# jakovdev/SequenceAligner

Hardware: AMD Instinct MI355X
Metric: pair-alignments/sec (higher is better)
Workload: dtype u16x2; 1 GPU; cfg2: 10000 protein seqs x U[80,120], nw blosum62 {'gap_pen': 4}, all-vs-all packed triangular; pairs=49995000, cells=501594494441, parallelism=pair-range x1

## Files before the change

sequencealigner_amd/csrc/sa_context.hip:

```cpp
#include <algorithm>
#include <cmath>
#include <cstdio>
#include <cstdlib>
#include <cstring>

#include "sa_ctx.h"

bool sa_device_ready(int device)
{
	int count = 0;
	hipError_t err = hipGetDeviceCount(&count);
	if (err != hipSuccess || count <= 0) {
		sa_set_error("No HIP devices available (%s); libseqalign_hip has no CPU fallback",
			     err == hipSuccess ? "device count is 0" : hipGetErrorString(err));
		return false;
	}
	if (device < 0 || device >= count) {
		sa_set_error("HIP device %d out of range (%d visible)", device, count);
		return false;
	}
	SA_HIP_CHECK(hipSetDevice(device), return false);
	return true;
}

// ... 237 lines not shown
	return sa_guard("sa_ctx_create", (sa_ctx *)nullptr, [&] { return ctx_create_impl(device, in, sc); });
}

extern "C" void sa_ctx_destroy(sa_ctx *ctx)
{
	if (!ctx)
		return;
	(void)hipSetDevice(ctx->device);
	for (auto &ev : ctx->events) {
		(void)hipEventDestroy(ev.e0);
		(void)hipEventDestroy(ev.e1);
	}
	sa_plan_release(ctx);
	sa_deliver_release(ctx);
	for (auto &ar : ctx->arranged) {
		(void)hipFree(ar.d_codes);
		(void)hipFree(ar.d_off);
		(void)hipFree(ar.d_rowmap);
		(void)hipFree(ar.d_posmap);
		(void)hipFree(ar.d_tok);
		(void)hipFree(ar.d_tok_off);
		(void)hipFree(ar.d_mine);
		(void)hipFree(ar.d_any);
	}
	(void)hipFree(ctx->d_codes);
	(void)hipFree(ctx->d_meta);
	(void)hipFree(ctx->d_off);
	(void)hipFree(ctx->d_sub);
	(void)hipFree(ctx->d_sub8);
	(void)hipFree(ctx->d_scratch);
	(void)hipFree(ctx->d_id_scratch);
	(void)hipFree(ctx->d_counters);
	for (hipEvent_t ev : ctx->slot_done)
		if (ev)
			(void)hipEventDestroy(ev);
	(void)hipFree(ctx->d_long_scratch);
	delete ctx;
}

extern "C" int64_t sa_ctx_pairs(const sa_ctx *ctx) { return ctx ? ctx->pairs : -1; }
bool sa_arranged_store(sa_ctx *ctx, const SaArrKey &key, const sa_ctx::Arranged **out)
{
	*out = nullptr;
	for (const auto &ar : ctx->arranged)
		if (ar.key == key) {
			*out = &ar;
// ... 24 lines not shown
		return false;
	sa_ctx::Arranged ar;
	ar.key = key;
	bool ok = false;
	do {
		if (!ts.tok.empty()) {
			SA_HIP_CHECK(hipMalloc(&ar.d_tok, sizeof(uint16_t) * ts.tok.size()), break);
			SA_HIP_CHECK(hipMalloc(&ar.d_tok_off, sizeof(int32_t) * ts.tok_off.size()), break);
			SA_HIP_CHECK(hipMalloc(&ar.d_mine, sizeof(uint16_t) * ts.mine.size()), break);
			SA_HIP_CHECK(hipMalloc(&ar.d_any, sizeof(uint16_t) * ts.any.size()), break);
			SA_HIP_CHECK(hipMemcpy(ar.d_tok, ts.tok.data(), sizeof(uint16_t) * ts.tok.size(), hipMemcpyHostToDevice), break);
			SA_HIP_CHECK(hipMemcpy(ar.d_tok_off, ts.tok_off.data(), sizeof(int32_t) * ts.tok_off.size(), hipMemcpyHostToDevice), break);
			SA_HIP_CHECK(hipMemcpy(ar.d_mine, ts.mine.data(), sizeof(uint16_t) * ts.mine.size(), hipMemcpyHostToDevice), break);
			SA_HIP_CHECK(hipMemcpy(ar.d_any, ts.any.data(), sizeof(uint16_t) * ts.any.size(), hipMemcpyHostToDevice), break);
		}
		SA_HIP_CHECK(hipMalloc(&ar.d_codes, codes_s.size()), break);
		SA_HIP_CHECK(hipMalloc(&ar.d_off, sizeof(int32_t) * off_s.size()), break);
		SA_HIP_CHECK(hipMalloc(&ar.d_rowmap, sizeof(int32_t) * rowmap.size()), break);
		SA_HIP_CHECK(hipMalloc(&ar.d_posmap, sizeof(int32_t) * posmap.size()), break);
		SA_HIP_CHECK(hipMemcpy(ar.d_codes, codes_s.data(), codes_s.size(), hipMemcpyHostToDevice), break);
		SA_HIP_CHECK(hipMemcpy(ar.d_off, off_s.data(), sizeof(int32_t) * off_s.size(), hipMemcpyHostToDevice), break);
		SA_HIP_CHECK(hipMemcpy(ar.d_rowmap, rowmap.data(), sizeof(int32_t) * rowmap.size(), hipMemcpyHostToDevice), break);
		SA_HIP_CHECK(hipMemcpy(ar.d_posmap, posmap.data(), sizeof(int32_t) * posmap.size(), hipMemcpyHostToDevice), break);
		ctx->arranged.push_back(ar);
		ok = true;
	} while (0);
	if (!ok) {
		(void)hipFree(ar.d_codes);
		(void)hipFree(ar.d_off);
		(void)hipFree(ar.d_rowmap);
		(void)hipFree(ar.d_posmap);
		(void)hipFree(ar.d_tok);
		(void)hipFree(ar.d_tok_off);
		(void)hipFree(ar.d_mine);
		(void)hipFree(ar.d_any);
		return false;
	}
	*out = &ctx->arranged.back();
	return true;
}

extern "C" void sa_ctx_timing(sa_ctx *ctx, int enable)
{
	if (!ctx)
		return;
	(void)hipSetDevice(ctx->device);
	for (auto &ev : ctx->events) {
		(void)hipEventDestroy(ev.e0);
		(void)hipEventDestroy(ev.e1);
	}
	ctx->events.clear();
	ctx->timing = enable != 0;
}

static int timing_read_impl(sa_ctx *ctx, char *kernel_name, int cap, int64_t *launches, double *total_ms,
			    int64_t *pairs, int64_t *cells, double *all_kernels_ms)
{
	if (!ctx)
		return 1;
	(void)hipSetDevice(ctx->device);
	struct Acc {
// ... 48 lines not shown
```

sequencealigner_amd/csrc/sa_ctx.h:

```cpp
#ifndef SA_CTX_H
#define SA_CTX_H

#include <atomic>
#include <chrono>
#include <deque>
#include <exception>
#include <memory>
#include <new>
#include <string>
#include <vector>

#include "sa_env.h"
#include "sa_guard.h"
#include "sa_internal.h"
#include "sa_plan.h"

struct sa_ctx {
	int device = 0;
	int32_t num = 0, max_len = 0, min_len = 0;
	int64_t pairs = 0;
	sa_scoring sc{};
	SaEnv env;
	std::vector<sa_meta> meta;
	std::vector<int32_t> off;
// ... 10 lines not shown
	enum { COUNTER_SLOTS = 256, COUNTERS_PER_SLOT = 2 * SA_PLAN_NCLASSES };
	unsigned *d_counters = nullptr;
	uint64_t call_no = 0;
	hipEvent_t slot_done[COUNTER_SLOTS] = {};
	bool slot_dirty[COUNTER_SLOTS] = {};
	int32_t *d_long_scratch = nullptr;
	int64_t long_stride = 0;
	int long_wgs = 0;
	int persistent_wgs = 0;
	bool sys_ok = false;
	int32_t sys_pconst = 0, sys_q = 0;
	int64_t sys_gain = 0, sys_slack = 0;
	int pk_kmax = 0, pk16_kmax = 0;
	int pk16_f16_kmax = 0;
	int pk_chunk_cap = SA_SYS_CHUNK;
	int32_t pk_pconst = 0, pk_q = 0, pk_floor = 0;
	int64_t pk_gain = 0, pk_slack = 0, pk_extra = 0;
	struct Arranged {
		SaArrKey key;
		uint8_t *d_codes = nullptr;
		int32_t *d_off = nullptr, *d_rowmap = nullptr, *d_posmap = nullptr;
		uint16_t *d_tok = nullptr, *d_mine = nullptr, *d_any = nullptr;
		int32_t *d_tok_off = nullptr;
	};
	std::deque<Arranged> arranged;
	int64_t tok_lean = 0, tok_legacy = 0;
	bool out_is_host = false;
	struct Plan {
		SaHostPlan h;
		struct DevClass {
			int32_t *d_jlist = nullptr, *d_tprefix = nullptr, *d_tlist = nullptr;
			int64_t *d_doff = nullptr;
		};
		struct DevBundle {
			SaPkClassArgs *d_args = nullptr;
			uint32_t *d_ulist = nullptr;
		};
		std::vector<DevClass> dc;
		std::vector<DevBundle> db;
		SaPlaceSeg *d_segs = nullptr;
		int32_t nsegs = 0;
		uint64_t stamp = 0;
	};
	std::vector<std::unique_ptr<Plan>> plans;
	Plan *plan = nullptr;
	uint64_t plan_clock = 0;
// ... 14 lines not shown
		double encode = 0, device = 0, upload = 0, code_objects = 0, pin = 0, plan = 0, arrange = 0;
	} setup;
	struct Deliver {
		hipStream_t compute = nullptr, copy = nullptr;
		hipEvent_t done[2] = {}, copied[2] = {};
		int32_t *d_buf[2] = {};
		int64_t buf_elems[2] = {};
		int32_t *h_stage[2] = {};
		int64_t stage_elems[2] = {};
		int32_t *d_packed = nullptr, *d_full = nullptr;
		int64_t packed_elems = 0, full_elems = 0;
		unsigned *h_counters = nullptr;
		int64_t h_counters_n = 0;
	} dl;
};

static inline double sa_ms_since(std::chrono::steady_clock::time_point t0)
{
	return std::chrono::duration<double, std::milli>(std::chrono::steady_clock::now() - t0).count();
}

bool sa_device_ready(int device);
bool sa_arranged_store(sa_ctx *ctx, const SaArrKey &key, const sa_ctx::Arranged **out);
SaPlanInputs sa_plan_inputs(const sa_ctx *ctx);

void sa_plan_release(sa_ctx *ctx);
bool sa_plan_get(sa_ctx *ctx, int64_t start, int64_t count, int world, bool share_host);
bool sa_prepare_range(sa_ctx *ctx, int64_t start, int64_t count, bool host_out);
int sa_align_range_impl(sa_ctx *ctx, int64_t start, int64_t count, int32_t *d_scores, void *stream, bool out16,
			int world = 0, int rank = 0, int32_t *host_out = nullptr);

void sa_deliver_release(sa_ctx *ctx);
bool sa_host_range_is_pinned(const void *p, size_t bytes);
size_t sa_host_available_bytes();
bool sa_host_range_in_malloc_heap(const void *p, size_t bytes);

bool sa_progress_wanted();
void sa_report_progress(double fraction);
void sa_progress_speaker(bool here);
int sa_devices_in_use(const SaEnv &env);

bool sa_align_gathered(struct sa_input in, struct sa_output out, const struct sa_scoring *sc, const int *devices, int ndev,
		       double *phase_seconds, double *breakdown_ms);
bool sa_rccl_available(std::string *why);

bool sa_norm_check(const char *who, const struct sa_norm *norm);
// ... 7 lines not shown
```

sequencealigner_amd/csrc/sa_launch.hip:

```cpp
#include <algorithm>
#include <cstdio>
#include <cstring>

#include "sa_ctx.h"


static void plan_free_device(sa_ctx::Plan &pl)
{
	for (auto &c : pl.dc) {
		(void)hipFree(c.d_jlist);
		(void)hipFree(c.d_tprefix);
		(void)hipFree(c.d_tlist);
		(void)hipFree(c.d_doff);
	}
	(void)hipFree(pl.d_segs);
	for (auto &b : pl.db) {
		(void)hipFree(b.d_args);
		(void)hipFree(b.d_ulist);
	}
	pl.dc.clear();
	pl.db.clear();
	pl.d_segs = nullptr;
}

void sa_plan_release(sa_ctx *ctx)
{
	for (auto &pl : ctx->plans)
		plan_free_device(*pl);
	ctx->plans.clear();
	ctx->plan = nullptr;
}

template <typename T> static bool upload(T *&dst, const std::vector<T> &v)
{
	SA_HIP_CHECK(hipMalloc(reinterpret_cast<void **>(&dst), sizeof(T) * std::max<size_t>(v.size(), 1)), return false);
	if (!v.empty()) {
		SA_HIP_CHECK(hipMemcpy(dst, v.data(), sizeof(T) * v.size(), hipMemcpyHostToDevice), return false);
	}
	return true;
}

static bool resolve_levels(sa_ctx *ctx, const SaArrKey (&keys)[SA_PK_SORT_LEVELS], SaArranged (&lv)[SA_PK_SORT_LEVELS])
{
	for (int l = 0; l < SA_PK_SORT_LEVELS; l++) {
		lv[l] = SaArranged{};
		if (!keys[l].block)
			continue;
		const sa_ctx::Arranged *ar = nullptr;
		if (!sa_arranged_store(ctx, keys[l], &ar))
			return false;
		if (ar)
			lv[l] = { ar->d_codes, ar->d_off, ar->d_rowmap, ar->d_posmap, ar->key.block, ar->d_tok, ar->d_tok_off, ar->d_mine, ar->d_any };
	}
	return true;
}

static bool plan_upload(sa_ctx *ctx, sa_ctx::Plan &pl)
{
	const SaHostPlan &h = pl.h;
	pl.dc.resize(h.classes.size());
	for (size_t ci = 0; ci < h.classes.size(); ci++) {
		const auto &cl = h.classes[ci];
		auto &d = pl.dc[ci];
		if (!upload(d.d_jlist, cl.jlist) || !upload(d.d_tprefix, cl.tprefix))
			return false;
		if (h.world >= 1 && (!upload(d.d_tlist, cl.tlist) || !upload(d.d_doff, cl.doff)))
			return false;
	}
	if (h.world >= 1 && !h.segs.empty()) {
		std::vector<SaPlaceSeg> segs(h.segs.size());
		for (size_t k = 0; k < h.segs.size(); k++) {
			const SaHostSeg &hs = h.segs[k];
			SaPlaceSeg &sg = segs[k];
			sg = SaPlaceSeg{};
			sg.src = hs.src;
// ... 7 lines not shown
			if (hs.map_kind) {
				const sa_ctx::Arranged *ar = nullptr;
				if (!sa_arranged_store(ctx, hs.key, &ar))
					return false;
				if (!ar) {
					sa_set_error("plan: placement names an arranged copy the store does not have");
					return false;
				}
				sg.map = hs.map_kind == 2 ? ar->d_posmap : ar->d_rowmap;
			}
		}
		if (!upload(pl.d_segs, segs))
			return false;
		pl.nsegs = (int32_t)segs.size();
	}
	pl.db.resize(h.bundles.size());
	for (size_t bi = 0; bi < h.bundles.size(); bi++) {
		const auto &b = h.bundles[bi];
		std::vector<SaPkClassArgs> args(b.args.size());
		for (size_t x = 0; x < b.args.size(); x++) {
			const SaHostPkArgs &ha = b.args[x];
			SaPkClassArgs &a = args[x];
			a = SaPkClassArgs{};
			if (!resolve_levels(ctx, ha.lv, a.lv))
				return false;
			const auto &d = pl.dc[(size_t)ha.cls_index];
			a.jlist = d.d_jlist;
			a.tprefix = d.d_tprefix;
			a.dense_off = h.world >= 1 ? d.d_doff : nullptr;
			a.ncols = ha.ncols;
			a.npart = ha.npart;
			a.k = ha.k;
			a.delta = ha.delta;
			a.pk_base = ha.pk_base;
			a.chunk = ha.chunk;
		}
		if (!upload(pl.db[bi].d_args, args) || !upload(pl.db[bi].d_ulist, b.ulist))
			return false;
	}
	return true;
}

bool sa_plan_get(sa_ctx *ctx, int64_t start, int64_t count, int world, bool share_host)
{
	for (auto &pl : ctx->plans)
		if (pl->h.start == start && pl->h.count == count && pl->h.world == world && pl->h.share_host == share_host) {
			pl->stamp = ++ctx->plan_clock;
// ... 544 lines not shown
```

sequencealigner_amd/csrc/sa_plan.cpp:

```cpp
#include "sa_plan.h"
#include "sa_guard.h"

#include <algorithm>
#include <cmath>
#include <cstdlib>

int32_t sa_column_of(int64_t p)
{
	int64_t j = (int64_t)((1.0 + std::sqrt(1.0 + 8.0 * (double)p)) * 0.5);
	while (j * (j - 1) / 2 > p)
		--j;
	while ((j + 1) * j / 2 <= p)
		++j;
	return (int32_t)j;
}

SaPairPlan::SaPairPlan(const sa_meta *m, int32_t n) : num(n), pairs((int64_t)n * (n - 1) / 2), meta(m)
{
	len_prefix.assign((size_t)n + 1, 0);
	cell_prefix.assign((size_t)n + 1, 0);
	for (int32_t k = 0; k < n; k++) {
		len_prefix[(size_t)k + 1] = len_prefix[(size_t)k] + m[k].len;
		cell_prefix[(size_t)k + 1] = cell_prefix[(size_t)k] + (int64_t)m[k].len * len_prefix[(size_t)k];
	}
// ... 133 lines not shown
			sa_set_error("token streams: store too large for 32-bit stream offsets");
			return false;
		}
	}
	ts.tok_off[(size_t)streams] = (int32_t)total;
	ts.tok.assign((size_t)total, (uint16_t)SA_CODE_NOP);
	ts.mine.assign((size_t)(total / 16), 0);
	ts.any.assign((size_t)(total / 16 / ng), 0);
	for (int32_t s = 0; s < streams; s++) {
		const int32_t b = off[(size_t)s * ch], n = off[(size_t)(s + 1) * ch] - b, at = ts.tok_off[(size_t)s];
		const int32_t any_at = ts.tok_off[(size_t)(s / ng * ng)] / 16 / ng;
		for (int32_t p = 0; p < n; p++) {
			const uint8_t c = codes[(size_t)b + (size_t)p];
			ts.tok[(size_t)at + (size_t)p] = c;
			if (c == SA_CODE_SEP) {
				ts.mine[(size_t)(at / 16 + p / 16)] |= (uint16_t)(1u << (p & 15));
				ts.any[(size_t)(any_at + p / 16)] |= (uint16_t)(1u << (p & 15));
			}
		}
	}
	return true;
}

static const char *const TOO_LARGE = "packed range too large for one launch; split it into smaller ranges";

bool sa_plan_host(const SaPlanInputs &in, int64_t start, int64_t count, int world, bool share_host, SaHostPlan &plan)
{
	plan = SaHostPlan();
	const int32_t num = in.num;
	const int64_t all_pairs = (int64_t)num * (num - 1) / 2;
	if (num < 2 || !in.meta || start < 0 || count <= 0 || start > all_pairs - count || world < 0 || world > 1024) {
		sa_set_error("plan: bad range [%lld,+%lld) of %lld pairs or world %d", (long long)start, (long long)count,
			     (long long)all_pairs, world);
		return false;
	}
	const int64_t end = start + count;
	std::vector<std::vector<int32_t>> jl((size_t)SA_PLAN_NCLASSES), tp((size_t)SA_PLAN_NCLASSES);
	std::vector<int64_t> cpairs((size_t)SA_PLAN_NCLASSES, 0), ccells((size_t)SA_PLAN_NCLASSES, 0);
	std::vector<std::vector<std::pair<int32_t, int32_t>>> rows_of((size_t)SA_PLAN_NCLASSES);
	std::vector<int64_t> lenpre((size_t)num + 1, 0);
	for (int32_t k = 0; k < num; k++)
		lenpre[(size_t)k + 1] = lenpre[(size_t)k] + in.meta[k].len;
	{
		const int64_t want_tiles = (int64_t)in.persistent_wgs * 6;
		const int64_t mine = world > 1 ? count / world : count;
		int32_t chunk = SA_SYS_CHUNK;
		while (chunk > 8 && mine / (4 * chunk) < want_tiles)
// ... 423 lines not shown
```

sequencealigner_amd/csrc/sa_plan.h:

```cpp
#ifndef SA_PLAN_H
#define SA_PLAN_H

#include <cstdint>
#include <string>
#include <utility>
#include <vector>

#include "sa_shapes.h"

int32_t sa_column_of(int64_t p);
inline int64_t sa_tri(int64_t j) { return j * (j - 1) / 2; }

struct SaPairPlan {
	int32_t num = 0;
	int64_t pairs = 0;
	const sa_meta *meta = nullptr;
	std::vector<int64_t> len_prefix;
	std::vector<int64_t> cell_prefix;
	SaPairPlan(const sa_meta *m, int32_t n);
	int64_t cells_before(int64_t p) const;
};

struct SaArrKey {
	int ng = 0, ch = 0;
// ... 31 lines not shown

int32_t sa_pk_delta(const SaPlanInputs &in, int g, int k);
int32_t sa_pk_base(const SaPlanInputs &in, int g, int k);

struct SaPkCls {
	bool small;
	int g, k;
};
SaPkCls sa_pk_decode(int cls);
int sa_systolic_class_for(int32_t n);

bool sa_arranged_exists(int32_t num, const SaArrKey &key);
int sa_pk_arranged_keys(const SaPlanInputs &in, int pk_g, int pk_k, int32_t chunk_pk, bool host_out, SaArrKey (&lv)[SA_PK_SORT_LEVELS]);
void sa_arrange_rows(const sa_meta *meta, int32_t num, const SaArrKey &key, std::vector<int32_t> &rowmap);

struct SaTokenStreams {
	int32_t streams = 0;
	std::vector<uint16_t> tok, mine, any;
	std::vector<int32_t> tok_off;
};
inline int32_t sa_token_blocks(int32_t smax, int g) { return ((smax + g - 1 + 15) >> 4) + 2; }
bool sa_build_tokens(const uint8_t *codes, const int32_t *off, int32_t num, const SaArrKey &key, SaTokenStreams &ts);

struct SaHostClass {
	int cls = 0;
	int32_t ncols = 0, ntiles = 0;
	int32_t npart = 0;
	int32_t chunk = 0;
	int64_t pairs = 0, cells = 0;
	std::vector<int32_t> jlist, tprefix;
	std::vector<int32_t> part_rows;
	std::vector<int32_t> tlist;
	std::vector<int64_t> doff;
	std::vector<int16_t> owner;
	std::vector<int32_t> rank_first;
	std::vector<int64_t> rank_pairs, rank_cells;
};

struct SaHostSeg {
	int64_t src, dst;
	int32_t count, pos0, ia, ib, flags;
	int map_kind;
	SaArrKey key;
};

struct SaHostPkArgs {
// ... 40 lines not shown
```

sequencealigner_amd/csrc/sa_shapes.h:

```cpp
#ifndef SA_SHAPES_H
#define SA_SHAPES_H

#include <cstdint>

#include "../../include/seqalign_hip.h"

#if defined(__HIPCC__)
#define SA_HD __host__ __device__
#else
#define SA_HD
#endif

enum : int { SA_CODE_SEP = 24, SA_CODE_NOP = 25, SA_CODE_ROWS = 26 };

void sa_set_error(const char *fmt, ...) __attribute__((format(printf, 1, 2)));


#define SA_SYS_CHUNK 32
#define SA_SYS_WPB(G, LONG) ((G) >= 32 ? 4 : 1)
#define SA_SYS_CLASS_LIST(X) \
	X(0, 8, 1) X(1, 8, 2) X(2, 8, 3) X(3, 8, 4) \
	X(4, 8, 5) X(5, 8, 6) X(6, 8, 7) X(7, 8, 8) \
	X(8, 8, 9) X(9, 8, 10) X(10, 8, 11) X(11, 8, 12) \
	X(12, 8, 13) X(13, 8, 14) X(14, 8, 15) X(15, 8, 16) \
// ... 23 lines not shown
}
#define SA_PK_F16_MAX 0x7bff
#define SA_PK_ROWS_OWN_BLOCK 1024
#define SA_PK_SORT_LEVELS 4
#define SA_PK_SORT_ROWS 2048
#define SA_PK_KMAX 24
#define SA_PK_K_LIST(X) \
	X(1) X(2) X(3) X(4) X(5) X(6) X(7) X(8) X(9) X(10) X(11) X(12) \
	X(13) X(14) X(15) X(16) X(17) X(18) X(19) X(20) X(21) X(22) X(23) X(24)
#define SA_PK_K16_MIN 13
#define SA_PK16_KMAX 64
#define SA_PK16_F16_KMAX 52
#define SA_PK_K16_LIST(X) \
	X(13) X(14) X(15) X(16) X(17) X(18) X(19) X(20) X(21) X(22) X(23) X(24) X(25) X(26) \
	X(27) X(28) X(29) X(30) X(31) X(32) X(33) X(34) X(35) X(36) X(37) X(38) X(39) X(40) \
	X(41) X(42) X(43) X(44) X(45) X(46) X(47) X(48) X(49) X(50) X(51) X(52) X(53) X(54) \
	X(55) X(56) X(57) X(58) X(59) X(60) X(61) X(62) X(63) X(64)
enum : int { SA_PK_CLASS0 = SA_SYS_NCLASSES + 1, SA_PK16_CLASS0 = SA_PK_CLASS0 + SA_PK_KMAX + 1,
	     SA_PK_CLASSES_END = SA_PK16_CLASS0 + SA_PK16_KMAX + 1,
	     SA_PK_SMALL = SA_PK_CLASSES_END - SA_PK_CLASS0,
	     SA_PLAN_NCLASSES = SA_PK_CLASSES_END + SA_PK_SMALL };

#define SA_PK_BUNDLE 8
struct SaArranged {
	const uint8_t *codes;
	const int32_t *off;
	const int32_t *rowmap;
	const int32_t *posmap;
	int32_t rows;
	const uint16_t *tok;
	const int32_t *tok_off;
	const uint16_t *mine;
	const uint16_t *any;
};
struct SaPkClassArgs {
	const int32_t *jlist;
	const int32_t *tprefix;
	const int64_t *dense_off;
	int32_t ncols, npart, k;
	int32_t delta, pk_base;
	int32_t chunk;
	SaArranged lv[SA_PK_SORT_LEVELS];
};
#define SA_PK_UTILE_BITS 28
SA_HD constexpr int sa_pk_lds_fixed(int g, int wpb) { return 416 * wpb * (64 / g); }
SA_HD constexpr int sa_pk_lds_bytes(int method, int g, int k) { return sa_pk_lds_fixed(g, sa_pk_wpb(method, g, k)) + SA_CODE_ROWS * ((k + 3) / 4) * 256; }
inline int sa_pk_bundle_klo(int g, int k) { return g == 8 ? 1 + (k - 1) / SA_PK_BUNDLE * SA_PK_BUNDLE : SA_PK_K16_MIN + (k - SA_PK_K16_MIN) / SA_PK_BUNDLE * SA_PK_BUNDLE; }


#define SA_SHARE_PAD(rows) (((rows) + 7) & ~7)

SA_HD inline int sa_pk_pick_level(const int32_t *lvrows, int32_t ra, int32_t rb, int32_t i_begin, int32_t tile_rows)
{
	int pick = -1;
	if (ra % tile_rows != 0)
		return pick;
// ... 22 lines not shown
```

sequencealigner_amd/csrc/sa_systolic_pk.inc:

```
#include "sa_internal.h"
#include <atomic>
#include <type_traits>
#if !defined(SA_PK_G) || (SA_PK_G != 8 && SA_PK_G != 16)
#error "define SA_PK_G (8 or 16) before including sa_systolic_pk.inc"
#endif
#if SA_PK_G == 16 && !defined(SA_PK16_PART)
#error "define SA_PK16_PART (0: K = 13..44, 1: K = 45..64) before including sa_systolic_pk.inc with SA_PK_G 16"
#endif

#define SA_PK_STORE(nt, v, p)                          \
	do {                                           \
		if (nt) {                              \
			asm volatile("");  \
			__builtin_nontemporal_store((v), (p)); \
		} else                                 \
			*(p) = (v);                    \
	} while (0)

#ifndef SA_PK_OPAQUE_TOKEN
#define SA_PK_OPAQUE_TOKEN 1
#endif
#ifndef SA_PK_PAIRED_ADDS
#define SA_PK_PAIRED_ADDS 1
#endif
// ... 156 lines not shown
	for (int h = 0; h < 2; h++) {
		const int32_t j = jh[h];
		tri[h] = (int64_t)j * (j - 1) / 2;
		const int64_t a = A.start > tri[h] ? A.start - tri[h] : 0;
		const int64_t b = A.end - tri[h] < j ? A.end - tri[h] : j;
		ia[h] = (int32_t)a;
		ib[h] = (int32_t)(b > a ? b : a);
		offj[h] = uload(A.off + j);
		nh[h] = uload(A.off + j + 1) - offj[h] - 1;
		pad[h] = W - nh[h];
	}
	const int32_t ra = ia[0] < ia[1] ? ia[0] : ia[1], rb = ib[0] > ib[1] ? ib[0] : ib[1];
	const int32_t chunk = t < nfull ? t - uload(A.tprefix + lo) : uload(A.tprefix + lo + 1) - uload(A.tprefix + lo);
	const int32_t ch_full = A.chunk;
	const int32_t i_begin = ra + chunk * (NGW * ch_full);
	const int32_t i_count = rb - i_begin < NGW * ch_full ? rb - i_begin : NGW * ch_full;
	const int32_t ch = (i_count + NGW - 1) / NGW;
	const int gw = wv * NG;
	const uint8_t *rcodes = A.codes;
	const int32_t *roff = A.off, *rowmap = nullptr, *posmap = nullptr;
	int32_t sort_rows = 0;
	const uint16_t *tk_tok = nullptr, *tk_mine = nullptr, *tk_any = nullptr;
	const int32_t *tk_off = nullptr;
	{
		const int32_t lvrows[SA_PK_SORT_LEVELS] = { uload(&A.lvp[0].rows), uload(&A.lvp[1].rows), uload(&A.lvp[2].rows),
							    uload(&A.lvp[3].rows) };
		static_assert(SA_PK_SORT_LEVELS == 4, "lvrows lists four levels");
		const int l = sa_pk_pick_level(lvrows, ra, rb, i_begin, NGW * ch_full);
		if (l >= 0) {
			const SaArranged &L = A.lvp[l];
			rcodes = uniform_ptr(L.codes);
			roff = uniform_ptr(L.off);
			rowmap = uniform_ptr(L.rowmap);
			posmap = uniform_ptr(L.posmap);
			tk_tok = uniform_ptr(L.tok);
			tk_off = uniform_ptr(L.tok_off);
			tk_mine = uniform_ptr(L.mine);
			tk_any = uniform_ptr(L.any);
			sort_rows = lvrows[0];
#pragma unroll
			for (int k = 1; k < SA_PK_SORT_LEVELS; k++)
				if (l == k)
					sort_rows = lvrows[k];
		}
	}
	const bool sorted = sort_rows > 0;

	int8_t *const sub = reinterpret_cast<int8_t *>(s_out_all);
	for (int k = lane_id; k < SA_SUB_DIM * SA_SUB_DIM; k += 64 * WPB)
		sub[k] = A.sub8[k];
	uint8_t *const s_cols = reinterpret_cast<uint8_t *>(s_ring_all);
	static_assert(2 * W <= WPB * NG * GSTRIDE * 2, "the staged columns fit the ring storage");
	for (int k = lane_id; k < 2 * W; k += 64 * WPB) {
		const int h = k >= W, c0 = k - h * W - pad[h];
		s_cols[k] = c0 >= 0 ? A.codes[offj[h] + c0] : (uint8_t)0xff;
	}
	__syncthreads();

	{
		constexpr int BUILDERS = NGW / COPIES;
		constexpr int ROWS_EACH = (SA_CODE_ROWS + BUILDERS - 1) / BUILDERS;
// ... 69 lines not shown
	auto fold16 = [&](unsigned long long m) -> uint32_t {
		m |= m >> 32;
		m |= m >> 16;
		return (uint32_t)m & 0xffffu;
	};
	auto block_events = [&](const uint32_t (&w)[TPL], uint32_t &mine) -> uint32_t {
		if (G == 16) {
			const unsigned long long m = __ballot(w[0] == SEPWORD);
			mine = (uint32_t)(m >> (lane & 48)) & 0xffffu;
			return fold16(m);
		}
		uint32_t any = 0;
		mine = 0;
#pragma unroll
		for (int u = 0; u < TPL; u++) {
			const unsigned long long m = __ballot(w[u] == SEPWORD);
			const uint32_t f = fold16(m);
			any |= ((f | (f >> 1)) & 0x5555u) << u;
			mine |= ((uint32_t)(m >> ((lane & 48) + (lane & 1))) & 0x5555u) << u;
		}
		return any;
	};

	const int32_t lean = __builtin_amdgcn_readfirstlane(tk_tok != nullptr ? 1 : 0);
	const uint16_t *tk_any_w = nullptr;
	if (lean) {
		const int32_t s0 = i_begin / ch_full + gw;
		const uint32_t o_w = (uint32_t)uload(tk_off + s0), o_g = (uint32_t)tk_off[s0 + grp];
		bw_a = 2u * o_g + (G == 8 ? 4u * (uint32_t)(r16 >> 1) : 2u * (uint32_t)r16);
		bw_b = o_g >> 3;
		tk_any_w = tk_any + (o_w >> 4) / NG;
		bw_c = (uint32_t)(WPB * OUT_HALFS * 2 + 2 * (wv * (NG * GSTRIDE) + grp * GSTRIDE + fpos(0)));
	}
	auto lean_load = [&](int32_t blk) -> uint32_t {
		const uint8_t *const b = reinterpret_cast<const uint8_t *>(tk_tok) + (size_t)(uint32_t)(blk << 5);
		asm volatile("" : "+v"(bw_a));
		return *reinterpret_cast<const tok_t *>(b + bw_a);
	};
	auto lean_mine = [&](int32_t blk) -> uint32_t {
		const uint8_t *const b = reinterpret_cast<const uint8_t *>(tk_mine) + (size_t)(uint32_t)(blk << 1);
		asm volatile("" : "+v"(bw_b));
		return *reinterpret_cast<const uint16_t *>(b + bw_b);
	};
	auto lean_any = [&](int32_t blk) -> uint32_t { return (uint32_t)tk_any_w[blk]; };
	auto lean_any_s = [&](uint32_t v) -> uint32_t { return (uint32_t)__builtin_amdgcn_readfirstlane((int)v); };
	auto lean_ring = [&](int32_t blk, uint32_t raw) {
		const uint32_t w = __umul24(raw, TUNIT);
		tok_t *const at = reinterpret_cast<tok_t *>(sa_pk_lds + bw_c + ((blk & 3) << 5));
		at[0] = (tok_t)w;
		at[RING * 2 / sizeof(tok_t)] = (tok_t)w;
	};

	const uint32_t base2 = pk2((uint32_t)A.pk_base);
	const uint32_t delta2 = pk2((uint32_t)A.delta);
	const uint32_t q2 = pk2((uint32_t)-A.q);
	const uint32_t cmask2 = (pad[0] == 0 ? 0xffffu : 0u) | (pad[1] == 0 ? 0xffff0000u : 0u);
	uint32_t V[K], Y[K];
	uint32_t vl[2];
	constexpr bool PAIRED = SA_PK_PAIRED_ADDS && METHOD == SA_METHOD_NW;
	uint32_t xout = 0;
	uint32_t vbase;
	uint32_t fl = 0;
	uint32_t flead = 0, xlead = 0;
	uint32_t best = 0, carry = 0;
	const uint32_t e2 = pk2((uint32_t)-A.gap_e);
	const uint32_t gqs2 = pk2((uint32_t)(A.gap_e - A.gap_o));
	int32_t frame = 0;
	int nsep = 0;
// ... 4 lines not shown
		const uint32_t top = base2 - o2 - (uint32_t)lig * e2;
		vl[0] = base2 - o2 - e2;
		vl[1] = top;
		xout = top - e2;
		xlead = base2 - o2;
		flead = base2;
		fl = base2 - (uint32_t)(lig + 1) * e2;
		best = base2 - (uint32_t)lig * e2;
#pragma unroll
		for (int q = 0; q < K; q++)
			V[q] = top, Y[q] = top;
	} else if (METHOD == SA_METHOD_NW) {
#pragma unroll
		for (int q = 0; q < K; q++)
			V[q] = base2, Y[q] = 0;
	} else {
		xout = base2 - q2;
#pragma unroll
		for (int q = 0; q < K; q++)
			V[q] = inj0, Y[q] = inj0;
	}

	__syncthreads();
	for (int k = lane; k < NG * GSTRIDE; k += 64)
		s_ring[k] = (uint16_t)NOPWORD;
	__syncthreads();
	uint32_t ev_lo = METHOD == SA_METHOD_GA ? 0x8000u : 0u, ev_hi;
	uint32_t gm, gmask;
	if (lean) {
		lean_ring(0, lean_load(0));
		gmask = lean_mine(0);
		ev_hi = lean_any_s(lean_any(0));
		gm = (gmask << 2) | (METHOD == SA_METHOD_GA ? 2u : 0u);
	} else {
		uint32_t w0[TPL];
#pragma unroll
		for (int u = 0; u < TPL; u++) {
			w0[u] = block_word(0, load_block(0, u), u);
			ring_write(0, w0[u], u);
		}
		ev_hi = block_events(w0, gmask);
		gm = (gmask << 2) | (METHOD == SA_METHOD_GA ? 2u : 0u);
	}
	int raw_next[TPL];
	uint32_t mask_pf = 0, any_next = 0;
	uint32_t &mask_next = TPL == 2 ? reinterpret_cast<uint32_t &>(raw_next[TPL - 1]) : mask_pf;
	if (lean) {
		raw_next[0] = (int)lean_load(1);
		mask_next = lean_mine(1);
		any_next = lean_any(1);
	} else {
#pragma unroll
		for (int u = 0; u < TPL; u++)
			raw_next[u] = load_block(1, u);
	}
	const uint8_t *const lane_prof = s_prof + copy * (NSLOT * 16) + lig * 16;
	auto ring_base = [&](int32_t blk) -> const uint16_t * { return ring + (((blk << 4) - lig) & (RING - 1)); };
	auto prof_row = [&](uint32_t word, uint4 (&P)[PARTS]) {
		const uint8_t *row = lane_prof + (word << TSHIFT);
#pragma unroll
		for (int p = 0; p < PARTS; p++)
			P[p] = *reinterpret_cast<const uint4 *>(row + p * PARTSTRIDE);
	};
	const uint16_t *rb0 = ring_base(0);
	uint32_t tk_cur = rb0[0], tk_nxt = rb0[1];
	uint4 P[PARTS];
	prof_row(tk_cur, P);

	auto do_block = [&](const int32_t blk) __attribute__((always_inline)) {
		if (A.rotate_prio) {
			switch (((uint32_t)A.rotate_prio + (uint32_t)blk) & 3u) {
			case 0: __builtin_amdgcn_s_setprio(0); break;
			case 1: __builtin_amdgcn_s_setprio(1); break;
			case 2: __builtin_amdgcn_s_setprio(2); break;
			default: __builtin_amdgcn_s_setprio(3); break;
			}
		}
		const uint32_t ev_in =
			METHOD == SA_METHOD_GA ? (ev_hi | (ev_hi << 1) | (ev_hi << 2) | (ev_lo >> 15) | (ev_lo >> 14)) : ev_hi;
		const uint32_t ev = ((ev_lo >> (16 - (G - 1))) | (ev_hi << (G - 1)) | ev_in) & 0xffffu;
		uint32_t gm_next, evn;
		__builtin_amdgcn_s_waitcnt(0x0f70);
		if (lean) {
			lean_ring(blk + 1, (uint32_t)raw_next[0]);
			gm_next = (mask_next << 2) | (gm >> 16);
			evn = lean_any_s(any_next);
			asm volatile("" ::: "memory");
			raw_next[0] = (int)lean_load(blk + 2);
			mask_next = lean_mine(blk + 2);
			any_next = lean_any(blk + 2);
		} else {
			uint32_t gmask_next;
			uint32_t wn[TPL];
#pragma unroll
			for (int u = 0; u < TPL; u++) {
				wn[u] = block_word(blk + 1, raw_next[u], u);
				ring_write(blk + 1, wn[u], u);
			}
			evn = block_events(wn, gmask_next);
			gm_next = (gmask_next << 2) | (gm >> 16);
#pragma unroll
			for (int u = 0; u < TPL; u++)
				raw_next[u] = load_block(blk + 2, u);
		}
		const uint16_t *rbase = ring_base(blk);

		auto step = [&](auto has_events, const int s) __attribute__((always_inline)) {
			uint32_t &vcur = vl[PAIRED ? 0 : s & 1];
			if (METHOD == SA_METHOD_SW)
				carry = pkmax(shift_in<G>(0u, carry), best);
			if (decltype(has_events)::value && __builtin_expect((ev >> s) & 1u, 0)) {
				asm volatile("" ::: "memory");
				if ((gm >> (s + 2)) & 1u) {
#pragma unroll
					for (int q = 0; q < K; q++) {
						V[q] = pksubsat(V[q], delta2);
						if (METHOD != SA_METHOD_NW)
							Y[q] = pksubsat(Y[q], delta2);
					}
					if (METHOD != SA_METHOD_NW)
						xout = pksubsat(xout, delta2);
					if (METHOD == SA_METHOD_SW) {
						fl = pksubsat(fl, delta2);
						best = pksubsat(best, delta2);
						carry = pksubsat(carry, delta2);
					}
					if (!leader) {
						vl[0] = pksubsat(vl[0], delta2);
						if (!PAIRED)
							vl[1] = pksubsat(vl[1], delta2);
					}
					frame++;
				}
				if (METHOD == SA_METHOD_GA && leader) {
					if ((gm >> (s + 2)) & 1u) {
						vl[(s + 1) & 1] = vbase;
						vcur = vbase + q2;
					} else if ((gm >> (s + 1)) & 1u) {
						vl[(s + 1) & 1] = vbase + (q2 & cmask2);
					} else if ((gm >> s) & 1u) {
						vcur = vbase;
					}
				}
				if (lig == G - 1 && tk_cur == SEPWORD) {
					const uint32_t v = METHOD == SA_METHOD_SW ? carry : V[K - 1];
					const int32_t rebase = (frame - nsep) * A.delta - A.pk_base +
							       (METHOD == SA_METHOD_SW ? ((blk << 4) + s - (G - 1)) * A.gap_e : 0);
					s_out[grp * CH + nsep] = (int16_t)((int32_t)(v & 0xffffu) + rebase);
					s_out[NG * CH + grp * CH + nsep] = (int16_t)((int32_t)(v >> 16) + rebase);
					nsep++;
				}
			}
			const uint32_t tk_far = rbase[s + 2];
			const uint32_t vprev = vl[PAIRED ? 0 : (s + 1) & 1];
			const uint8_t *const row_next = lane_prof + (tk_nxt << TSHIFT);
			auto reload = [&](int q_done) {
				if ((q_done & 3) == 3 || q_done == K - 1) {
					P[q_done >> 2] = *reinterpret_cast<const uint4 *>(row_next + (q_done >> 2) * PARTSTRIDE);
					if ((K & 3) != 0 && (q_done >> 2) == PARTS - 1)
						asm volatile("" ::"v"(P[PARTS - 1].y), "v"(P[PARTS - 1].z), "v"(P[PARTS - 1].w));
				}
			};
			uint32_t dnw[K];
			if (METHOD == SA_METHOD_NW) {
				if (PAIRED) {
#pragma unroll
					for (int q = 0; q + 1 < K; q += 2)
						pkadd2(q ? V[q - 1] : vprev, V[q], comp(P[q >> 2], q & 3), comp(P[q >> 2], (q & 3) + 1), dnw[q], dnw[q + 1]);
					if (K & 1)
						dnw[K - 1] = (K > 1 ? V[K > 1 ? K - 2 : 0] : vprev) + comp(P[(K - 1) >> 2], (K - 1) & 3);
				} else {
					dnw[0] = vprev + comp(P[0], 0);
#pragma unroll
					for (int q = 1; q < K; q++)
						dnw[q] = V[q - 1] + comp(P[q >> 2], q & 3);
				}
#pragma unroll
				for (int p = 0; p < PARTS; p++)
// ... 107 lines not shown
					uint32_t t0;
					{
						const uint32_t y = pkmax(V[0], Y[0]);
						Y[0] = y;
						t0 = pkmax(vprev + comp(P[0], 0), y);
						if (K == 1)
							reload(0);
					}
#pragma unroll
					for (int q = 0; q < K; q++) {
						const uint32_t m = pkmax(t0, x);
						if (q + 1 < K) {
							const uint32_t y = pkmax(V[q + 1], Y[q + 1]);
							Y[q + 1] = y;
							t0 = pkmax(V[q] + comp(P[(q + 1) >> 2], (q + 1) & 3), y);
							reload(q + 1);
						}
						V[q] = m - q2;
						x = pkmax(V[q], x);
					}
				}
				xout = x;
			}
			tk_cur = tk_nxt;
#if SA_PK_OPAQUE_TOKEN
			uint32_t tk_wide = tk_far;
			asm volatile("" : "+v"(tk_wide));
			tk_nxt = tk_wide;
#else
			tk_nxt = tk_far;
#endif
		};
		constexpr bool QUIET = SA_PK_QUIET_BLOCKS && METHOD == SA_METHOD_NW && G == 8 && K <= 16;
		if (QUIET && ev == 0) {
#pragma unroll
			for (int s = 0; s < 16; s++)
				step(std::false_type{}, s);
		} else {
#pragma unroll
			for (int s = 0; s < 16; s++)
				step(std::true_type{}, s);
		}
		gm = gm_next;
		ev_lo = ev_hi;
		ev_hi = evn;
	};
	const unsigned long long ph1 = A.stamps ? __builtin_amdgcn_s_memtime() : 0ull;
	for (int32_t blk2 = 0; blk2 < nblk; blk2 += 2) {
		do_block(blk2);
		if (blk2 + 1 < nblk)
			do_block(blk2 + 1);
	}
	if (A.stamps && threadIdx.x == 0) {
		A.stamps[3 * (size_t)A.nlocal + 3 * (size_t)A.stamp_u + 0] = ph1;
		A.stamps[3 * (size_t)A.nlocal + 3 * (size_t)A.stamp_u + 1] = __builtin_amdgcn_s_memtime();
		A.stamps[3 * (size_t)A.nlocal + 3 * (size_t)A.stamp_u + 2] = (unsigned long long)nblk * 16;
	}
	__syncthreads();

	if (A.dense_off) {
		const int64_t draw = A.dense_off[t];
		const int64_t dbase = (int64_t)(((uint64_t)(uint32_t)__builtin_amdgcn_readfirstlane((int32_t)(draw >> 32)) << 32) |
						(uint32_t)__builtin_amdgcn_readfirstlane((int32_t)draw));
		const int32_t cntp = SA_SHARE_PAD(i_count);
#pragma unroll
		for (int g = 0; g < NG; g++) {
			int32_t c = i_count - (gw + g) * ch;
			c = c < 0 ? 0 : c > ch ? ch : c;
			if (lane < c && active) {
				const int32_t is = i_begin + (gw + g) * ch + lane;
				const int32_t m = roff[is + 1] - roff[is] - 1;
#pragma unroll
				for (int h = 0; h < 2; h++) {
					if (h == 1 && dup)
// ... 264 lines not shown
```

Before: 4.005 billion pair-alignments/s.

## Stream pre-scaled token row offsets into registers instead of an LDS ring

Adds a per-stride host-built row stream of pre-multiplied profile byte offsets for each token. For NW with G=8 and K<=16, the systolic kernel loads 16 tokens per block straight into registers as uint4 vectors. This replaces the LDS token ring and its waitcnt barrier, and mask/any loads become direct global reads. The cost is extra device memory, host setup to build the row streams, and more vector registers per lane.

```diff
diff --git a/sequencealigner_amd/csrc/sa_context.hip b/sequencealigner_amd/csrc/sa_context.hip
--- a/sequencealigner_amd/csrc/sa_context.hip
+++ b/sequencealigner_amd/csrc/sa_context.hip
@@ -283,6 +283,8 @@
 		(void)hipFree(ar.d_tok_off);
 		(void)hipFree(ar.d_mine);
 		(void)hipFree(ar.d_any);
+		for (auto &r : ar.rows)
+			(void)hipFree(r.d_rows);
 	}
 	(void)hipFree(ctx->d_codes);
 	(void)hipFree(ctx->d_meta);
@@ -353,7 +355,10 @@
 		SA_HIP_CHECK(hipMemcpy(ar.d_off, off_s.data(), sizeof(int32_t) * off_s.size(), hipMemcpyHostToDevice), break);
 		SA_HIP_CHECK(hipMemcpy(ar.d_rowmap, rowmap.data(), sizeof(int32_t) * rowmap.size(), hipMemcpyHostToDevice), break);
 		SA_HIP_CHECK(hipMemcpy(ar.d_posmap, posmap.data(), sizeof(int32_t) * posmap.size(), hipMemcpyHostToDevice), break);
-		ctx->arranged.push_back(ar);
+		ar.h_tok.streams = ts.streams;
+		ar.h_tok.tok = std::move(ts.tok);
+		ar.h_tok.tok_off = std::move(ts.tok_off);
+		ctx->arranged.push_back(std::move(ar));
 		ok = true;
 	} while (0);
 	if (!ok) {
@@ -368,6 +373,34 @@
 		return false;
 	}
 	*out = &ctx->arranged.back();
+	return true;
+}
+
+bool sa_arranged_rows(sa_ctx *ctx, const sa_ctx::Arranged *ar_in, uint32_t stride, const uint32_t **out)
+{
+	*out = nullptr;
+	sa_ctx::Arranged *ar = nullptr;
+	for (auto &a : ctx->arranged)
+		if (&a == ar_in)
+			ar = &a;
+	if (!ar || !ar->d_tok)
+		return true;
+	for (const auto &r : ar->rows)
+		if (r.stride == stride) {
+			*out = r.d_rows;
+			return true;
+		}
+	const auto t_arr = std::chrono::steady_clock::now();
+	std::vector<uint32_t> rows;
+	if (!sa_build_row_streams(ar->h_tok, ar->key.ng, stride, rows))
+		return false;
+	sa_ctx::Arranged::Rows r;
+	r.stride = stride;
+	SA_HIP_CHECK(hipMalloc(&r.d_rows, sizeof(uint32_t) * rows.size()), return false);
+	SA_HIP_CHECK(hipMemcpy(r.d_rows, rows.data(), sizeof(uint32_t) * rows.size(), hipMemcpyHostToDevice), (void)hipFree(r.d_rows); return false);
+	ar->rows.push_back(r);
+	ctx->setup.arrange += sa_ms_since(t_arr);
+	*out = r.d_rows;
 	return true;
 }
 
diff --git a/sequencealigner_amd/csrc/sa_ctx.h b/sequencealigner_amd/csrc/sa_ctx.h
--- a/sequencealigner_amd/csrc/sa_ctx.h
+++ b/sequencealigner_amd/csrc/sa_ctx.h
@@ -56,6 +56,12 @@
 		int32_t *d_off = nullptr, *d_rowmap = nullptr, *d_posmap = nullptr;
 		uint16_t *d_tok = nullptr, *d_mine = nullptr, *d_any = nullptr;
 		int32_t *d_tok_off = nullptr;
+		struct Rows {
+			uint32_t stride = 0;
+			uint32_t *d_rows = nullptr;
+		};
+		std::vector<Rows> rows;
+		SaTokenStreams h_tok;
 	};
 	std::deque<Arranged> arranged;
 	int64_t tok_lean = 0, tok_legacy = 0;
@@ -116,6 +122,7 @@
 
 bool sa_device_ready(int device);
 bool sa_arranged_store(sa_ctx *ctx, const SaArrKey &key, const sa_ctx::Arranged **out);
+bool sa_arranged_rows(sa_ctx *ctx, const sa_ctx::Arranged *ar, uint32_t stride, const uint32_t **out);
 SaPlanInputs sa_plan_inputs(const sa_ctx *ctx);
 
 void sa_plan_release(sa_ctx *ctx);
diff --git a/sequencealigner_amd/csrc/sa_launch.hip b/sequencealigner_amd/csrc/sa_launch.hip
--- a/sequencealigner_amd/csrc/sa_launch.hip
+++ b/sequencealigner_amd/csrc/sa_launch.hip
@@ -40,7 +40,7 @@
 	return true;
 }
 
-static bool resolve_levels(sa_ctx *ctx, const SaArrKey (&keys)[SA_PK_SORT_LEVELS], SaArranged (&lv)[SA_PK_SORT_LEVELS])
+static bool resolve_levels(sa_ctx *ctx, const SaArrKey (&keys)[SA_PK_SORT_LEVELS], uint32_t row_stride, SaArranged (&lv)[SA_PK_SORT_LEVELS])
 {
 	for (int l = 0; l < SA_PK_SORT_LEVELS; l++) {
 		lv[l] = SaArranged{};
@@ -49,8 +49,12 @@
 		const sa_ctx::Arranged *ar = nullptr;
 		if (!sa_arranged_store(ctx, keys[l], &ar))
 			return false;
-		if (ar)
-			lv[l] = { ar->d_codes, ar->d_off, ar->d_rowmap, ar->d_posmap, ar->key.block, ar->d_tok, ar->d_tok_off, ar->d_mine, ar->d_any };
+		if (!ar)
+			continue;
+		const uint32_t *rowoff = nullptr;
+		if (row_stride && !sa_arranged_rows(ctx, ar, row_stride, &rowoff))
+			return false;
+		lv[l] = { ar->d_codes, ar->d_off, ar->d_rowmap, ar->d_posmap, ar->key.block, ar->d_tok, ar->d_tok_off, ar->d_mine, ar->d_any, rowoff };
 	}
 	return true;
 }
@@ -104,7 +108,7 @@
 			const SaHostPkArgs &ha = b.args[x];
 			SaPkClassArgs &a = args[x];
 			a = SaPkClassArgs{};
-			if (!resolve_levels(ctx, ha.lv, a.lv))
+			if (!resolve_levels(ctx, ha.lv, sa_pk_reg_tokens(ctx->sc.method, b.g, ha.k) ? sa_pk_row_stride(ha.k) : 0u, a.lv))
 				return false;
 			const auto &d = pl.dc[(size_t)ha.cls_index];
 			a.jlist = d.d_jlist;
diff --git a/sequencealigner_amd/csrc/sa_plan.cpp b/sequencealigner_amd/csrc/sa_plan.cpp
--- a/sequencealigner_amd/csrc/sa_plan.cpp
+++ b/sequencealigner_amd/csrc/sa_plan.cpp
@@ -179,7 +179,38 @@
 	return true;
 }
 
-static const char *const TOO_LARGE = "packed range too large for one launch; split it into smaller ranges";
+bool sa_build_row_streams(const SaTokenStreams &ts, int ng, uint32_t stride, std::vector<uint32_t> &rows)
+{
+	rows.clear();
+	if (ts.streams <= 0)
+		return true;
+	if (ng <= 0 || 64 % ng != 0 || ts.streams % ng != 0 || ts.tok_off.size() != (size_t)ts.streams + 1 || stride == 0) {
+		sa_set_error("row streams: %d streams in slots of %d, stride %u", ts.streams, ng, stride);
+		return false;
+	}
+	const int g = 64 / ng;
+	const int64_t total = sa_row_stream_at(ts.tok_off[(size_t)ts.streams], ts.streams) - SA_ROW_FRONT;
+	if (total * 4 > (int64_t)1 << 31) {
+		sa_set_error("row streams: store too large for 32-bit byte offsets");
+		return false;
+	}
+	rows.assign((size_t)total, (uint32_t)SA_CODE_NOP * stride);
+	for (int32_t s = 0; s < ts.streams; s++) {
+		const int32_t at = ts.tok_off[(size_t)s], padded = ts.tok_off[(size_t)s + 1] - at;
+		const int64_t p0 = sa_row_stream_at(at, s);
+		const int64_t lo = p0 - SA_ROW_FRONT, hi = sa_row_stream_at(ts.tok_off[(size_t)s + 1], s + 1) - SA_ROW_FRONT;
+		const int32_t nblk = padded / 16 - 2;
+		if (padded % 16 != 0 || nblk < 1 || p0 - (g - 1) < lo || p0 + 16 * (nblk + 1) + 15 >= hi || lo < 0 || hi > total) {
+			sa_set_error("row streams: the windows of stream %d (%d positions, %d-lane groups) leave its region", s, padded, g);
+			return false;
+		}
+		for (int32_t p = 0; p < padded; p++)
+			rows[(size_t)(p0 + p)] = (uint32_t)ts.tok[(size_t)at + (size_t)p] * stride;
+	}
+	return true;
+}
+
+static const char *const TOO_LARGE ="packed range too large for one launch; split it into smaller ranges";
 
 bool sa_plan_host(const SaPlanInputs &in, int64_t start, int64_t count, int world, bool share_host, SaHostPlan &plan)
 {
diff --git a/sequencealigner_amd/csrc/sa_plan.h b/sequencealigner_amd/csrc/sa_plan.h
--- a/sequencealigner_amd/csrc/sa_plan.h
+++ b/sequencealigner_amd/csrc/sa_plan.h
@@ -77,6 +77,9 @@
 inline int32_t sa_token_blocks(int32_t smax, int g) { return ((smax + g - 1 + 15) >> 4) + 2; }
 bool sa_build_tokens(const uint8_t *codes, const int32_t *off, int32_t num, const SaArrKey &key, SaTokenStreams &ts);
 
+inline int64_t sa_row_stream_at(int32_t tok_off, int32_t stream) { return (int64_t)tok_off + (int64_t)SA_ROW_FRONT * (stream + 1); }
+bool sa_build_row_streams(const SaTokenStreams &ts, int ng, uint32_t stride, std::vector<uint32_t> &rows);
+
 struct SaHostClass {
 	int cls = 0;
 	int32_t ncols = 0, ntiles = 0;
diff --git a/sequencealigner_amd/csrc/sa_shapes.h b/sequencealigner_amd/csrc/sa_shapes.h
--- a/sequencealigner_amd/csrc/sa_shapes.h
+++ b/sequencealigner_amd/csrc/sa_shapes.h
@@ -69,6 +69,12 @@
 	     SA_PLAN_NCLASSES = SA_PK_CLASSES_END + SA_PK_SMALL };
 
 #define SA_PK_BUNDLE 8
+#ifndef SA_PK_REG_TOKENS
+#define SA_PK_REG_TOKENS 1
+#endif
+SA_HD constexpr bool sa_pk_reg_tokens(int method, int g, int k) { return SA_PK_REG_TOKENS && method == SA_METHOD_NW && g == 8 && k <= 16; }
+#define SA_ROW_FRONT 16
+SA_HD constexpr uint32_t sa_pk_row_stride(int k) { return (uint32_t)((k + 3) / 4) * 256u; }
 struct SaArranged {
 	const uint8_t *codes;
 	const int32_t *off;
@@ -79,6 +85,7 @@
 	const int32_t *tok_off;
 	const uint16_t *mine;
 	const uint16_t *any;
+	const uint32_t *rowoff;
 };
 struct SaPkClassArgs {
 	const int32_t *jlist;
diff --git a/sequencealigner_amd/csrc/sa_systolic_pk.inc b/sequencealigner_amd/csrc/sa_systolic_pk.inc
--- a/sequencealigner_amd/csrc/sa_systolic_pk.inc
+++ b/sequencealigner_amd/csrc/sa_systolic_pk.inc
@@ -202,6 +202,7 @@
 	int32_t sort_rows = 0;
 	const uint16_t *tk_tok = nullptr, *tk_mine = nullptr, *tk_any = nullptr;
 	const int32_t *tk_off = nullptr;
+	const uint32_t *tk_rows = nullptr;
 	{
 		const int32_t lvrows[SA_PK_SORT_LEVELS] = { uload(&A.lvp[0].rows), uload(&A.lvp[1].rows), uload(&A.lvp[2].rows),
 							    uload(&A.lvp[3].rows) };
@@ -217,6 +218,7 @@
 			tk_off = uniform_ptr(L.tok_off);
 			tk_mine = uniform_ptr(L.mine);
 			tk_any = uniform_ptr(L.any);
+			tk_rows = uniform_ptr(L.rowoff);
 			sort_rows = lvrows[0];
 #pragma unroll
 			for (int k = 1; k < SA_PK_SORT_LEVELS; k++)
@@ -332,15 +334,21 @@
 		return any;
 	};
 
-	const int32_t lean = __builtin_amdgcn_readfirstlane(tk_tok != nullptr ? 1 : 0);
+	constexpr bool REGT = sa_pk_reg_tokens(METHOD, G, K);
+	static_assert(!REGT || TSHIFT == 0, "a row stream holds byte offsets");
+	const int32_t lean = __builtin_amdgcn_readfirstlane(tk_tok != nullptr && (!REGT || tk_rows != nullptr) ? 1 : 0);
 	const uint16_t *tk_any_w = nullptr;
 	if (lean) {
 		const int32_t s0 = i_begin / ch_full + gw;
 		const uint32_t o_w = (uint32_t)uload(tk_off + s0), o_g = (uint32_t)tk_off[s0 + grp];
-		bw_a = 2u * o_g + (G == 8 ? 4u * (uint32_t)(r16 >> 1) : 2u * (uint32_t)r16);
 		bw_b = o_g >> 3;
 		tk_any_w = tk_any + (o_w >> 4) / NG;
-		bw_c = (uint32_t)(WPB * OUT_HALFS * 2 + 2 * (wv * (NG * GSTRIDE) + grp * GSTRIDE + fpos(0)));
+		if (REGT) {
+			bw_a = 4u * (o_g + (uint32_t)SA_ROW_FRONT * (uint32_t)(s0 + grp + 1) - (uint32_t)lig);
+		} else {
+			bw_a = 2u * o_g + (G == 8 ? 4u * (uint32_t)(r16 >> 1) : 2u * (uint32_t)r16);
+			bw_c = (uint32_t)(WPB * OUT_HALFS * 2 + 2 * (wv * (NG * GSTRIDE) + grp * GSTRIDE + fpos(0)));
+		}
 	}
 	auto lean_load = [&](int32_t blk) -> uint32_t {
 		const uint8_t *const b = reinterpret_cast<const uint8_t *>(tk_tok) + (size_t)(uint32_t)(blk << 5);
@@ -352,8 +360,22 @@
 		asm volatile("" : "+v"(bw_b));
 		return *reinterpret_cast<const uint16_t *>(b + bw_b);
 	};
+	typedef uint32_t u32x4_a4 __attribute__((ext_vector_type(4), aligned(4)));
+	typedef uint32_t u32_a2 __attribute__((aligned(2)));
+	auto reg_load = [&](int32_t blk, int qd) -> u32x4 {
+		const uint8_t *const b = reinterpret_cast<const uint8_t *>(tk_rows) + (size_t)(uint32_t)(blk << 6);
+		asm volatile("" : "+v"(bw_a));
+		return *reinterpret_cast<const u32x4_a4 *>(b + bw_a + 16 * qd);
+	};
+	auto reg_mine = [&](int32_t blk) -> uint32_t {
+		const uint8_t *const b = reinterpret_cast<const uint8_t *>(tk_mine) + (size_t)(uint32_t)((blk << 1) - 2);
+		asm volatile("" : "+v"(bw_b));
+		return *reinterpret_cast<const u32_a2 *>(b + bw_b);
+	};
 	auto lean_any = [&](int32_t blk) -> uint32_t { return (uint32_t)tk_any_w[blk]; };
 	auto lean_any_s = [&](uint32_t v) -> uint32_t { return (uint32_t)__builtin_amdgcn_readfirstlane((int)v); };
+	auto reg_any = [&](int32_t blk) -> uint32_t { return *reinterpret_cast<const u32_a2 *>(tk_any_w + (blk - 1)); };
+	auto reg_any_s = [&](uint32_t v) -> uint32_t { return (uint32_t)__builtin_amdgcn_readfirstlane((int)v) >> 16; };
 	auto lean_ring = [&](int32_t blk, uint32_t raw) {
 		const uint32_t w = __umul24(raw, TUNIT);
 		tok_t *const at = reinterpret_cast<tok_t *>(sa_pk_lds + bw_c + ((blk & 3) << 5));
@@ -404,12 +426,21 @@
 	}
 
 	__syncthreads();
-	for (int k = lane; k < NG * GSTRIDE; k += 64)
-		s_ring[k] = (uint16_t)NOPWORD;
+	if (!(REGT && lean))
+		for (int k = lane; k < NG * GSTRIDE; k += 64)
+			s_ring[k] = (uint16_t)NOPWORD;
 	__syncthreads();
 	uint32_t ev_lo = METHOD == SA_METHOD_GA ? 0x8000u : 0u, ev_hi;
 	uint32_t gm, gmask;
-	if (lean) {
+	u32x4 TQ[4] = {};
+	if (REGT && lean) {
+#pragma unroll
+		for (int qd = 0; qd < 4; qd++)
+			TQ[qd] = reg_load(0, qd);
+		gmask = lean_mine(0);
+		ev_hi = lean_any_s(lean_any(0));
+		gm = (gmask << 16) | (METHOD == SA_METHOD_GA ? 0x8000u : 0u);
+	} else if (lean) {
 		lean_ring(0, lean_load(0));
 		gmask = lean_mine(0);
 		ev_hi = lean_any_s(lean_any(0));
@@ -427,7 +458,9 @@
 	int raw_next[TPL];
 	uint32_t mask_pf = 0, any_next = 0;
 	uint32_t &mask_next = TPL == 2 ? reinterpret_cast<uint32_t &>(raw_next[TPL - 1]) : mask_pf;
-	if (lean) {
+	if (REGT && lean) {
+		any_next = reg_any(1);
+	} else if (lean) {
 		raw_next[0] = (int)lean_load(1);
 		mask_next = lean_mine(1);
 		any_next = lean_any(1);
@@ -444,12 +477,19 @@
 		for (int p = 0; p < PARTS; p++)
 			P[p] = *reinterpret_cast<const uint4 *>(row + p * PARTSTRIDE);
 	};
-	const uint16_t *rb0 = ring_base(0);
-	uint32_t tk_cur = rb0[0], tk_nxt = rb0[1];
+	uint32_t tk_cur = 0, tk_nxt = 0;
+	if (REGT && lean) {
+		tk_cur = TQ[0][0];
+	} else {
+		const uint16_t *rb0 = ring_base(0);
+		tk_cur = rb0[0], tk_nxt = rb0[1];
+	}
 	uint4 P[PARTS];
 	prof_row(tk_cur, P);
 
-	auto do_block = [&](const int32_t blk) __attribute__((always_inline)) {
+	auto do_block = [&](auto way, const int32_t blk) __attribute__((always_inline)) {
+		constexpr bool RW = decltype(way)::value;
+		constexpr int MB = RW ? 16 : 2;
 		if (A.rotate_prio) {
 			switch (((uint32_t)A.rotate_prio + (uint32_t)blk) & 3u) {
 			case 0: __builtin_amdgcn_s_setprio(0); break;
@@ -461,9 +501,15 @@
 		const uint32_t ev_in =
 			METHOD == SA_METHOD_GA ? (ev_hi | (ev_hi << 1) | (ev_hi << 2) | (ev_lo >> 15) | (ev_lo >> 14)) : ev_hi;
 		const uint32_t ev = ((ev_lo >> (16 - (G - 1))) | (ev_hi << (G - 1)) | ev_in) & 0xffffu;
-		uint32_t gm_next, evn;
-		__builtin_amdgcn_s_waitcnt(0x0f70);
-		if (lean) {
+		uint32_t gm_next = 0, evn;
+		if constexpr (!RW)
+			__builtin_amdgcn_s_waitcnt(0x0f70);
+		if constexpr (RW) {
+			evn = reg_any_s(any_next);
+			asm volatile("" ::: "memory");
+			mask_next = reg_mine(blk + 1);
+			any_next = reg_any(blk + 2);
+		} else if (!REGT && lean) {
 			lean_ring(blk + 1, (uint32_t)raw_next[0]);
 			gm_next = (mask_next << 2) | (gm >> 16);
 			evn = lean_any_s(any_next);
@@ -485,7 +531,8 @@
 			for (int u = 0; u < TPL; u++)
 				raw_next[u] = load_block(blk + 2, u);
 		}
-		const uint16_t *rbase = ring_base(blk);
+		const uint16_t *rbase = RW ? nullptr : ring_base(blk);
+		auto T = [&](int s) -> uint32_t { return TQ[(s >> 2) & 3][s & 3]; };
 
 		auto step = [&](auto has_events, const int s) __attribute__((always_inline)) {
 			uint32_t &vcur = vl[PAIRED ? 0 : s & 1];
@@ -493,7 +540,7 @@
 				carry = pkmax(shift_in<G>(0u, carry), best);
 			if (decltype(has_events)::value && __builtin_expect((ev >> s) & 1u, 0)) {
 				asm volatile("" ::: "memory");
-				if ((gm >> (s + 2)) & 1u) {
+				if ((gm >> (s + MB)) & 1u) {
 #pragma unroll
 					for (int q = 0; q < K; q++) {
 						V[q] = pksubsat(V[q], delta2);
@@ -515,16 +562,16 @@
 					frame++;
 				}
 				if (METHOD == SA_METHOD_GA && leader) {
-					if ((gm >> (s + 2)) & 1u) {
+					if ((gm >> (s + MB)) & 1u) {
 						vl[(s + 1) & 1] = vbase;
 						vcur = vbase + q2;
-					} else if ((gm >> (s + 1)) & 1u) {
+					} else if ((gm >> (s + MB - 1)) & 1u) {
 						vl[(s + 1) & 1] = vbase + (q2 & cmask2);
-					} else if ((gm >> s) & 1u) {
+					} else if ((gm >> (s + MB - 2)) & 1u) {
 						vcur = vbase;
 					}
 				}
-				if (lig == G - 1 && tk_cur == SEPWORD) {
+				if (lig == G - 1 && (RW ? T(s) : tk_cur) == SEPWORD) {
 					const uint32_t v = METHOD == SA_METHOD_SW ? carry : V[K - 1];
 					const int32_t rebase = (frame - nsep) * A.delta - A.pk_base +
 							       (METHOD == SA_METHOD_SW ? ((blk << 4) + s - (G - 1)) * A.gap_e : 0);
@@ -533,9 +580,11 @@
 					nsep++;
 				}
 			}
-			const uint32_t tk_far = rbase[s + 2];
+			uint32_t tk_far = 0;
+			if constexpr (!RW)
+				tk_far = rbase[s + 2];
 			const uint32_t vprev = vl[PAIRED ? 0 : (s + 1) & 1];
-			const uint8_t *const row_next = lane_prof + (tk_nxt << TSHIFT);
+			const uint8_t *const row_next = lane_prof + (RW ? T(s + 1) : tk_nxt << TSHIFT);
 			auto reload = [&](int q_done) {
 				if ((q_done & 3) == 3 || q_done == K - 1) {
 					P[q_done >> 2] = *reinterpret_cast<const uint4 *>(row_next + (q_done >> 2) * PARTSTRIDE);
@@ -689,6 +738,10 @@
 				}
 				xout = x;
 			}
+			if constexpr (RW) {
+				if ((s & 3) == 3)
+					TQ[s >> 2] = reg_load(blk + 1, s >> 2);
+			} else {
 			tk_cur = tk_nxt;
 #if SA_PK_OPAQUE_TOKEN
 			uint32_t tk_wide = tk_far;
@@ -697,6 +750,7 @@
 #else
 			tk_nxt = tk_far;
 #endif
+			}
 		};
 		constexpr bool QUIET = SA_PK_QUIET_BLOCKS && METHOD == SA_METHOD_NW && G == 8 && K <= 16;
 		if (QUIET && ev == 0) {
@@ -708,15 +762,27 @@
 			for (int s = 0; s < 16; s++)
 				step(std::true_type{}, s);
 		}
-		gm = gm_next;
+		if constexpr (RW)
+			gm = mask_next;
+		else
+			gm = gm_next;
 		ev_lo = ev_hi;
 		ev_hi = evn;
 	};
 	const unsigned long long ph1 = A.stamps ? __builtin_amdgcn_s_memtime() : 0ull;
-	for (int32_t blk2 = 0; blk2 < nblk; blk2 += 2) {
-		do_block(blk2);
-		if (blk2 + 1 < nblk)
-			do_block(blk2 + 1);
+	if (REGT && lean) {
+		if constexpr (REGT)
+			for (int32_t blk2 = 0; blk2 < nblk; blk2 += 2) {
+				do_block(std::true_type{}, blk2);
+				if (blk2 + 1 < nblk)
+					do_block(std::true_type{}, blk2 + 1);
+			}
+	} else {
+		for (int32_t blk2 = 0; blk2 < nblk; blk2 += 2) {
+			do_block(std::false_type{}, blk2);
+			if (blk2 + 1 < nblk)
+				do_block(std::false_type{}, blk2 + 1);
+		}
 	}
 	if (A.stamps && threadIdx.x == 0) {
 		A.stamps[3 * (size_t)A.nlocal + 3 * (size_t)A.stamp_u + 0] = ph1;
```

New measurement: 4.079 billion pair-alignments/s (median of 6 runs). 1.02x the previous value.
